# mmziyad/flink-ms

Hardware: AMD Instinct MI355X
Metric: ALS training throughput (ratings/sec per iteration) (higher is better)
Workload: dtype bf16+fp8-factors; 1 GPU; model=ALS-ml25m-shape, rank=64, ratings_per_gpu=25000095, users_per_gpu=162541, num_items=59047, global_batch=25000095, factor_exchange=fp8-e4m3, solve_dtype=fp32, parallelism=dp1+factor-allgather

## Files before the change

flink_ms_amd/ops/csrc/als_kernels.hip:

```cpp

#include "common.hip.h"

#include "als_kernels_device.inc"
#include "fma_api.h"


template <int KT, bool FP8, bool WT = false>
__launch_bounds__(256)
__attribute__((amdgpu_waves_per_eu(3)))
__global__ void k_als_solve_fused(
    const long long* __restrict__ indptr, const int* __restrict__ indices,
    const float* __restrict__ values,
    const typename GatherT<FP8>::elem* __restrict__ factors,
    float* __restrict__ out_f32,
    typename GatherT<FP8>::elem* __restrict__ out_lowp,
    const int* __restrict__ row_order, long long nrows, float reg,
    const float* __restrict__ scale, const float* __restrict__ G0) {
    constexpr int K = Geo<KT>::K;
    __shared__ __align__(16) char
        smem[FP8 ? Geo<KT>::SMEM8_TRI : Geo<KT>::SMEM_TRI];
    long long row = blockIdx.x;
    if (row >= nrows) return;
    if (row_order) row = row_order[row];

// ... 792 lines not shown
            const int row = I * 16 + g4 * 4 + r, col = J * 16 + li;
            if constexpr (I == J)
                T[t][r] = G0[max(row, col) * K + min(row, col)];
            else
                T[t][r] = G0[row * K + col];
        }
        wavefused_load_base<KT, t + 1>(T, G0, g4, li);
    }
}

template <int KT, bool FP8, int BC, bool WT = false>
__launch_bounds__(256)
__attribute__((amdgpu_waves_per_eu(5)))
__global__ void k_als_solve_wavefused(const long long* __restrict__ indptr,
                                      const int* __restrict__ indices,
                                      const float* __restrict__ values,
                                      const void* __restrict__ factors,
                                      float* __restrict__ out_f32,
                                      unsigned short* __restrict__ out_bf16,
                                      unsigned char* __restrict__ out_fp8,
                                      const int* __restrict__ row_order,
                                      long long nrows, float reg,
                                      const float* __restrict__ scale,
                                      const float* __restrict__ G0) {
    constexpr int K = KT * 16;
    static_assert(K <= 64, "wave-fused path handles k <= 64");
    constexpr int NA = KT * (KT + 1) / 2;
    constexpr int TROW = FP8 ? Geo<KT>::TROW8 : Geo<KT>::TROW;
    constexpr int SB = (K + 16) * TROW;
    constexpr int NT = FP8 ? 8 * (K / 16) : K;
    constexpr int NCHW = (2 * NT <= WAVE && NT >= 8) ? 2 : 1;
    constexpr int SCRF = (K * 17 > 1040) ? K * 17 : 1040;
    constexpr int WB0 = (NCHW * SB > SCRF * 4) ? NCHW * SB : SCRF * 4;
    constexpr int WB = (WB0 + 15) & ~15;
    __shared__ __align__(16) char smem[4 * WB];
    const int w = __builtin_amdgcn_readfirstlane(threadIdx.x >> 6);
    const int lane = threadIdx.x & 63;
    const long long e0 = (long long)blockIdx.x * 4 + w;
    if (e0 >= nrows) return;
    const long long e = row_order ? row_order[e0] : e0;
    char* buf = smem + (long long)w * WB;
    float* scr = (float*)buf;
    const int g4 = lane >> 4, li = lane & 15;
    const long long p0 = indptr[e];
    const int n = (int)(indptr[e + 1] - p0);
    if (n == 0) {
        if (lane < K) {
            out_f32[e * K + lane] = 0.0f;
            if (out_bf16) out_bf16[e * K + lane] = 0;
            if (out_fp8) out_fp8[e * K + lane] = 0;
        }
        return;
    }
    {
        constexpr int SEGS = FP8 ? 8 : 16;
        for (int i = lane; i < NCHW * 14 * SEGS; i += WAVE) {
            const int b = i / (14 * SEGS), r2 = i % (14 * SEGS);
            const int row = K + 2 + r2 / SEGS, seg = r2 % SEGS;
            *(unsigned*)(buf + b * SB + (long long)row * TROW + seg * 4) =
                0u;
        }
    }
    f32x4 T[NA], E[KT];
    if constexpr (WT) {
        wavefused_load_base<KT>(T, G0, g4, li);
    } else {
#pragma unroll
        for (int t = 0; t < NA; ++t) T[t] = f32x4{0, 0, 0, 0};
    }
#pragma unroll
    for (int p = 0; p < KT; ++p) E[p] = f32x4{0, 0, 0, 0};
    const int nchunks = (n + 31) >> 5;
    for (int ch = 0; ch < nchunks; ch += NCHW) {
        if constexpr (NCHW == 2) {
            const int sub = (lane >= NT) ? 1 : 0;
            const int lch = ch + sub;
            if (lch < nchunks && lane < 2 * NT)
                stage_chunk_w<KT, FP8, NT, WT>(buf + sub * SB, indices,
                                               values, factors,
                                               p0 + (long long)lch * 32,
                                               n - lch * 32, lane - sub * NT,
                                               scale);
        } else {
            stage_chunk_w<KT, FP8, WAVE, WT>(buf, indices, values, factors,
                                             p0 + (long long)ch * 32,
                                             n - ch * 32, lane, scale);
        }
        WREG_FENCE();
        {
            typename FragT<FP8>::type frag[KT + 1];
            read_frags<KT, FP8>(buf, lane, frag);
            mfma_lower_tiles<KT, FP8>(frag, T);
            mfma_ext_tiles<KT, FP8>(frag, E);
        }
        if constexpr (NCHW == 2) {
            if (ch + 1 < nchunks) {
                typename FragT<FP8>::type frag[KT + 1];
                read_frags<KT, FP8>(buf + SB, lane, frag);
                mfma_lower_tiles<KT, FP8>(frag, T);
                mfma_ext_tiles<KT, FP8>(frag, E);
            }
        }
        WREG_FENCE();
    }
    wavefused_dump_b<KT>(E, scr, g4, li);
    WREG_FENCE();
    float x0 = (lane < K) ? scr[lane] + scr[64 + lane] : 0.0f;
    WREG_FENCE();
    wavefused_diag<KT, BC>(T, reg, (float)n, g4, li);
    float d0 = 1.0f;
    wreg_panels<KT, 0, BC>(T, scr, lane, g4, li, d0);
    const float id0 = wreg_id0<BC>(d0);
    wreg_forward<KT, 0, BC>(T, scr, x0, id0, lane, g4, li);
    x0 *= id0;
    wreg_backward<KT, KT - 1, BC>(T, scr, x0, id0, lane, g4, li);
    x0 = wreg_canon_nan(x0);
    if (lane < K) {
        out_f32[e * K + lane] = x0;
        if (out_bf16) out_bf16[e * K + lane] = f2bf(x0);
        if (out_fp8) out_fp8[e * K + lane] = f2fp8(x0);
    }
}

template <int KT, int t = 0>
DEV_INLINE void factor_gram_store(const f32x4* T, float* dst, int g4, int li) {
    if constexpr (t < KT * (KT + 1) / 2) {
        constexpr int K = KT * 16;
        constexpr int I = lo_tile_i(t);
        constexpr int J = t - (I * (I + 1)) / 2;
#pragma unroll
        for (int r = 0; r < 4; ++r)
            dst[(I * 16 + g4 * 4 + r) * K + J * 16 + li] = T[t][r];
        factor_gram_store<KT, t + 1>(T, dst, g4, li);
    }
}
// ... 427 lines not shown
```

flink_ms_amd/ops/csrc/als_kernels_device.inc:

```
#pragma once

#include <type_traits>


template <int KT> struct Geo {
    static constexpr int K = 16 * KT;
    static constexpr int NA = KT * (KT + 1) / 2;
    static constexpr int TILES = NA + KT;
    static constexpr int SLOTS = (TILES + 3) / 4;
    static constexpr int TROW = 96;
    static constexpr int STAGE_BYTES = (K + 16) * TROW;
    static constexpr int TROW8 = 40;
    static constexpr int STAGE8_BYTES = (K + 16) * TROW8;
    static constexpr int NCH_BF16 = 2;
    static constexpr int NCH_FP8 = 4;
    static constexpr int STAGE_TOTAL = NCH_BF16 * STAGE_BYTES;
    static constexpr int STAGE8_TOTAL = NCH_FP8 * STAGE8_BYTES;
    static constexpr int A_BYTES = K * (K + 1) * 4;
    static constexpr int CHOL_BYTES = A_BYTES + 8 * K + 16 * 16 * 4;
    static constexpr int SMEM = (NCH_BF16 * STAGE_BYTES > CHOL_BYTES)
                                    ? NCH_BF16 * STAGE_BYTES : CHOL_BYTES;
    static constexpr int SMEM8 = (NCH_FP8 * STAGE8_BYTES > CHOL_BYTES)
                                     ? NCH_FP8 * STAGE8_BYTES : CHOL_BYTES;
    static constexpr int LDT = 17;
// ... 25 lines not shown

typedef float stage_f32x2 __attribute__((ext_vector_type(2)));
typedef __bf16 stage_bf16x2 __attribute__((ext_vector_type(2)));

DEV_INLINE float stage_fp8_sat(float x) {
    const unsigned u = __builtin_bit_cast(unsigned, x);
    return (u & 0x7f800000u) != 0x7f800000u
               ? __builtin_amdgcn_fmed3f(x, 448.0f, -448.0f) : x;
}

DEV_INLINE unsigned stage_rescale_fp8x4(unsigned w, float s) {
    const stage_f32x2 s2 = {s, s};
    stage_f32x2 lo = __builtin_amdgcn_cvt_pk_f32_fp8((int)w, false) * s2;
    stage_f32x2 hi = __builtin_amdgcn_cvt_pk_f32_fp8((int)w, true) * s2;
    int r = __builtin_amdgcn_cvt_pk_fp8_f32(stage_fp8_sat(lo.x),
                                            stage_fp8_sat(lo.y), 0, false);
    r = __builtin_amdgcn_cvt_pk_fp8_f32(stage_fp8_sat(hi.x),
                                        stage_fp8_sat(hi.y), r, true);
    return (unsigned)r;
}

DEV_INLINE unsigned stage_rescale_bf16x2(unsigned d, float s) {
    const stage_f32x2 v = {__builtin_bit_cast(float, d << 16),
                           __builtin_bit_cast(float, d & 0xffff0000u)};
    const stage_f32x2 s2 = {s, s};
    return __builtin_bit_cast(
        unsigned, __builtin_convertvector(v * s2, stage_bf16x2));
}

DEV_INLINE uint4 stage_widen_fp8x8(uint2 raw) {
    unsigned out[4];
#pragma unroll
    for (int h = 0; h < 4; ++h) {
        const unsigned w = (h < 2 ? raw.x : raw.y) >> (16 * (h & 1));
        out[h] = (unsigned)f2bf(fp82f((unsigned char)(w & 0xffu)))
                 | ((unsigned)f2bf(fp82f((unsigned char)((w >> 8) & 0xffu)))
                    << 16);
    }
    return uint4{out[0], out[1], out[2], out[3]};
}

template <bool FP8>
DEV_INLINE uint4 stage_rescale_piece(uint4 x, float s) {
    if constexpr (FP8)
        return uint4{stage_rescale_fp8x4(x.x, s), stage_rescale_fp8x4(x.y, s),
                     stage_rescale_fp8x4(x.z, s), stage_rescale_fp8x4(x.w, s)};
    else
        return uint4{stage_rescale_bf16x2(x.x, s),
                     stage_rescale_bf16x2(x.y, s),
                     stage_rescale_bf16x2(x.z, s),
                     stage_rescale_bf16x2(x.w, s)};
}

template <int KT, bool FP8, int NLANES = WAVE, bool WT = false,
          bool IDENT = false, bool WIDEN = false>
DEV_INLINE void stage_chunk_w(char* buf,
                              const int* __restrict__ indices,
                              const float* __restrict__ values,
                              const void* __restrict__ factors_v,
                              long long base, int nrem, int lane,
                              const float* __restrict__ scale = nullptr) {
    constexpr int K = Geo<KT>::K;
    constexpr int TROW = FP8 ? Geo<KT>::TROW8 : Geo<KT>::TROW;
    if constexpr (FP8) {
        const unsigned char* factors = (const unsigned char*)factors_v;
        constexpr int NT = 8 * (K / 16);
        for (int t = lane; t < NT; t += NLANES) {
            const int q = t & 7, c16 = t >> 3;
            uint4 v[4];
            [[maybe_unused]] float sc[4] = {0.0f, 0.0f, 0.0f, 0.0f};
#pragma unroll
            for (int m = 0; m < 4; ++m) {
                uint4 x = {0, 0, 0, 0};
                const int row = 4 * q + m;
                if (row < nrem) {
                    long long col;
                    if constexpr (IDENT) col = base + row;
                    else col = indices[base + row];
                    x = *(const uint4*)(factors + col * (long long)K
                                        + c16 * 16);
                    if constexpr (WT) sc[m] = scale[base + row];
                }
                v[m] = x;
            }
            if constexpr (WT) {
#pragma unroll
                for (int m = 0; m < 4; ++m)
                    v[m] = stage_rescale_piece<FP8>(v[m], sc[m]);
            }
            char* rb = buf + (long long)(16 * c16) * TROW + q * 4;
#pragma unroll
            for (int cc = 0; cc < 16; ++cc) {
                unsigned wd = 0;
#pragma unroll
                for (int m = 0; m < 4; ++m)
                    wd |= (((&v[m].x)[cc >> 2] >> (8 * (cc & 3))) & 0xffu)
                          << (8 * m);
                *(unsigned*)(rb + (long long)cc * TROW) = wd;
            }
        }
    } else {
        const unsigned short* factors = (const unsigned short*)factors_v;
        constexpr int NT = 8 * (K / 8);
        for (int t = lane; t < NT; t += NLANES) {
            const int q = t & 7, c8 = t >> 3;
            uint4 v[4];
            [[maybe_unused]] float sc[4] = {0.0f, 0.0f, 0.0f, 0.0f};
#pragma unroll
            for (int m = 0; m < 4; ++m) {
                uint4 x = {0, 0, 0, 0};
                const int row = 4 * q + m;
                if (row < nrem) {
                    long long col;
                    if constexpr (IDENT) col = base + row;
                    else col = indices[base + row];
                    if constexpr (WIDEN)
                        x = stage_widen_fp8x8(*(const uint2*)(
                            (const unsigned char*)factors_v
                            + col * (long long)K + c8 * 8));
                    else
                        x = *(const uint4*)(factors + col * (long long)K
                                            + c8 * 8);
                    if constexpr (WT) sc[m] = scale[base + row];
                }
                v[m] = x;
            }
            if constexpr (WT) {
#pragma unroll
                for (int m = 0; m < 4; ++m)
                    v[m] = stage_rescale_piece<FP8>(v[m], sc[m]);
            }
            char* rb = buf + (long long)(8 * c8) * TROW + q * 8;
#pragma unroll
            for (int cc = 0; cc < 8; ++cc) {
                const unsigned d0 = (&v[0].x)[cc >> 1], d1 = (&v[1].x)[cc >> 1];
                const unsigned d2 = (&v[2].x)[cc >> 1], d3 = (&v[3].x)[cc >> 1];
                unsigned lo, hi;
                if (cc & 1) {
                    lo = (d0 >> 16) | (d1 & 0xffff0000u);
                    hi = (d2 >> 16) | (d3 & 0xffff0000u);
                } else {
                    lo = (d0 & 0xffffu) | (d1 << 16);
                    hi = (d2 & 0xffffu) | (d3 << 16);
                }
                *(uint2*)(rb + (long long)cc * TROW) = uint2{lo, hi};
            }
        }
    }
    if constexpr (IDENT) return;
    if (lane < 8) {
        if constexpr (FP8) {
            unsigned h = 0, l = 0;
#pragma unroll
            for (int m = 0; m < 4; ++m) {
                const int row = 4 * lane + m;
                const float r = (row < nrem) ? values[base + row] : 0.0f;
                const unsigned char hb = f2fp8(r);
                const unsigned char lb = f2fp8(r - fp82f(hb));
                h |= ((unsigned)hb) << (8 * m);
                l |= ((unsigned)lb) << (8 * m);
            }
            *(unsigned*)(buf + (long long)K * TROW + lane * 4) = h;
            *(unsigned*)(buf + (long long)(K + 1) * TROW + lane * 4) = l;
        } else {
            unsigned h2[2] = {0, 0}, l2[2] = {0, 0};
#pragma unroll
            for (int m = 0; m < 4; ++m) {
                const int row = 4 * lane + m;
                const float r = (row < nrem) ? values[base + row] : 0.0f;
                const unsigned short h = f2bf(r);
                const unsigned short l = f2bf(r - bf2f(h));
                h2[m >> 1] |= ((unsigned)h) << (16 * (m & 1));
                l2[m >> 1] |= ((unsigned)l) << (16 * (m & 1));
            }
            *(uint2*)(buf + (long long)K * TROW + lane * 8) =
                uint2{h2[0], h2[1]};
            *(uint2*)(buf + (long long)(K + 1) * TROW + lane * 8) =
                uint2{l2[0], l2[1]};
        }
    }
}

template <int KT, bool FP8, int NCH>
DEV_INLINE void stage_zero_pad_all(char* smem) {
    constexpr int K = Geo<KT>::K;
    constexpr int TROW = FP8 ? Geo<KT>::TROW8 : Geo<KT>::TROW;
    constexpr int SB = (K + 16) * TROW;
    constexpr int SEGS = FP8 ? 8 : 16;
    for (int i = threadIdx.x; i < NCH * 14 * SEGS; i += 256) {
        const int b = i / (14 * SEGS), rem = i % (14 * SEGS);
        const int row = K + 2 + rem / SEGS, seg = rem % SEGS;
        *(unsigned*)(smem + (long long)b * SB + (long long)row * TROW
                     + seg * 4) = 0u;
    }
}

template <int KT, bool FP8>
DEV_INLINE void read_frags(const char* buf, int lane,
                           typename FragT<FP8>::type* frag) {
    constexpr int TROW = FP8 ? Geo<KT>::TROW8 : Geo<KT>::TROW;
    constexpr int FB = FP8 ? 8 : 16;
    const int g = lane >> 4, li = lane & 15;
#pragma unroll
    for (int t = 0; t <= KT; ++t)
        frag[t] = *(const typename FragT<FP8>::type*)(
            buf + (long long)(t * 16 + li) * TROW + g * FB);
}


template <int KT, int W, bool FP8, int S = 0>
DEV_INLINE void mfma_tiles(const typename FragT<FP8>::type* frag, f32x4* acc) {
    if constexpr (S < Geo<KT>::SLOTS) {
        constexpr int t = W + 4 * S;
        if constexpr (t < Geo<KT>::TILES) {
            constexpr int NA = Geo<KT>::NA;
            constexpr int p = (t < NA) ? up_tile_p(t, KT) : (t - NA);
            constexpr int q = (t < NA) ? up_tile_q((t < NA) ? t : 0, KT) : KT;
            if constexpr (FP8) {
                acc[S] = __builtin_amdgcn_mfma_f32_16x16x32_fp8_fp8(
                    frag[p], frag[q], acc[S], 0, 0, 0);
            } else {
                acc[S] = __builtin_amdgcn_mfma_f32_16x16x32_bf16(
                    frag[p], frag[q], acc[S], 0, 0, 0);
            }
        }
        mfma_tiles<KT, W, FP8, S + 1>(frag, acc);
    }
}

template <int KT, int W, int S = 0>
DEV_INLINE void write_acc(const f32x4* acc, float* A, float* bhi, float* blo,
                          int lane) {
    if constexpr (S < Geo<KT>::SLOTS) {
        constexpr int t = W + 4 * S;
        if constexpr (t < Geo<KT>::TILES) {
            constexpr int K = Geo<KT>::K;
            constexpr int NA = Geo<KT>::NA;
            constexpr int p = (t < NA) ? up_tile_p(t, KT) : (t - NA);
            constexpr int q = (t < NA) ? up_tile_q((t < NA) ? t : 0, KT) : KT;
            const int g = lane >> 4, li = lane & 15;
#pragma unroll
            for (int r = 0; r < 4; ++r) {
                const int row = p * 16 + g * 4 + r;
                if constexpr (q == KT) {
                    if (li == 0) bhi[row] = acc[S][r];
                    else if (li == 1) blo[row] = acc[S][r];
                } else {
// ... 201 lines not shown
        }
        __syncthreads();
        if (own && tid < B0) {
            const float* Tbr = A + tri_off(bi, Ir) * TSZ + lr;
            float s = 0.0f;
#pragma unroll
            for (int cc = 0; cc < 16; ++cc)
                s += Tbr[cc * LDT] * xbuf[B0 + cc];
            acc -= s * invd;
        } else if (own && tid >= B0 && tid < B0 + 16) {
            acc = xbuf[tid];
        }
        __syncthreads();
    }
    if (own) {
        x_row[tid] = acc;
        if (xb_row) xb_row[tid] = f2bf(acc);
        if (x8_row) x8_row[tid] = f2fp8(acc);
    }
}

template <int KT, bool COMBINE = true, bool TRI = false, bool FP8 = false,
          bool WT = false>
DEV_INLINE int gramian_to_lds(char* smem,
                              const long long* __restrict__ indptr,
                              const int* __restrict__ indices,
                              const float* __restrict__ values,
                              const void* __restrict__ factors,
                              long long row, float reg,
                              const float* __restrict__ scale = nullptr,
                              const float* __restrict__ G0 = nullptr) {
    constexpr int K = Geo<KT>::K;
    constexpr int NCH = FP8 ? Geo<KT>::NCH_FP8 : Geo<KT>::NCH_BF16;
    constexpr int SB = (K + 16) * (FP8 ? Geo<KT>::TROW8 : Geo<KT>::TROW);
    const int tid = threadIdx.x, lane = tid & 63;
    const int w = __builtin_amdgcn_readfirstlane(threadIdx.x >> 6);
    const long long p0 = indptr[row];
    const int n = (int)(indptr[row + 1] - p0);
    if (n == 0) return 0;

    f32x4 acc[Geo<KT>::SLOTS];
#pragma unroll
    for (int s = 0; s < Geo<KT>::SLOTS; ++s) acc[s] = f32x4{0, 0, 0, 0};

    constexpr int NT = FP8 ? 8 * (K / 16) : K;
    constexpr int TW = (NT > WAVE) ? 2 : 1;
    constexpr int NCHU = (NCH < 4 / TW) ? NCH : 4 / TW;
    stage_zero_pad_all<KT, FP8, NCHU>(smem);
    const int team = w / TW;
    const int tlane = (w % TW) * WAVE + lane;
    const int nchunks = (n + 31) >> 5;
    for (int r0 = 0; r0 < nchunks; r0 += NCHU) {
        if (team < NCHU && r0 + team < nchunks)
            stage_chunk_w<KT, FP8, TW * WAVE, WT>(
                smem + team * SB, indices, values, factors,
                p0 + (long long)(r0 + team) * 32, n - (r0 + team) * 32,
                tlane, scale);
        __syncthreads();
        const int ns = min(NCHU, nchunks - r0);
        for (int sc = 0; sc < ns; ++sc) {
            typename FragT<FP8>::type frag[KT + 1];
            read_frags<KT, FP8>(smem + sc * SB, lane, frag);
            switch (w) {
                case 0: mfma_tiles<KT, 0, FP8>(frag, acc); break;
                case 1: mfma_tiles<KT, 1, FP8>(frag, acc); break;
                case 2: mfma_tiles<KT, 2, FP8>(frag, acc); break;
                default: mfma_tiles<KT, 3, FP8>(frag, acc); break;
            }
        }
        __syncthreads();
    }

    float* A = (float*)smem;
    float* bhi = A + (TRI ? Geo<KT>::A_TRI_FLOATS : K * (K + 1));
    float* blo = bhi + K;
    if constexpr (TRI) {
        switch (w) {
            case 0: write_acc_tri<KT, 0>(acc, A, bhi, blo, lane); break;
            case 1: write_acc_tri<KT, 1>(acc, A, bhi, blo, lane); break;
            case 2: write_acc_tri<KT, 2>(acc, A, bhi, blo, lane); break;
            default: write_acc_tri<KT, 3>(acc, A, bhi, blo, lane); break;
        }
    } else {
        switch (w) {
            case 0: write_acc<KT, 0>(acc, A, bhi, blo, lane); break;
            case 1: write_acc<KT, 1>(acc, A, bhi, blo, lane); break;
            case 2: write_acc<KT, 2>(acc, A, bhi, blo, lane); break;
            default: write_acc<KT, 3>(acc, A, bhi, blo, lane); break;
        }
    }
    __syncthreads();
    if constexpr (WT && COMBINE) {
        if constexpr (TRI) {
            const int lr = tid >> 4, lc = tid & 15;
            int I = 0, J = 0;
            for (int t = 0; t < Geo<KT>::NA; ++t) {
                const int r = I * 16 + lr, c = J * 16 + lc;
                A[t * Geo<KT>::TSZ + lr * Geo<KT>::LDT + lc] +=
                    G0[max(r, c) * K + min(r, c)];
                if (++J > I) { ++I; J = 0; }
            }
        } else {
            for (int i = tid; i < K * K; i += 256) {
                const int r = i / K, c = i % K;
                A[r * (K + 1) + c] += G0[max(r, c) * K + min(r, c)];
            }
        }
// ... 33 lines not shown
```

flink_ms_amd/ops/csrc/bindings.cpp:

```cpp

#include <torch/extension.h>

#include <charconv>
#include <cstdint>
#include <cstdlib>
#include <thread>
#include <vector>

#include "fma_api.h"

namespace {

py::tuple parse_als_block(py::object text_o, int64_t k) {
    Py_buffer view;
    if (PyObject_GetBuffer(text_o.ptr(), &view, PyBUF_SIMPLE) != 0)
        throw py::error_already_set();
    char* base = (char*)view.buf;
    Py_ssize_t total = view.len;
    std::vector<std::pair<int64_t, int64_t>> lines;
    int64_t start = 0;
    for (int64_t i = 0; i < total; ++i) {
        if (base[i] == '\n') {
            if (i > start) lines.emplace_back(start, i);
            start = i + 1;
// ... 694 lines not shown
              a.name());
    return py::make_tuple(greater, equal, score);
}

int64_t rank_chunk_items(int64_t np, int64_t nc) {
    return (int64_t)fma_rank_chunk_items(np, nc);
}


void mfma_probe_f32(torch::Tensor A, torch::Tensor B, torch::Tensor D,
                    int64_t stream) {
    Args a("mfma_probe_f32");
    a.flat(A, kF32, "A", 16 * 4, true);
    a.flat(B, kF32, "B", 4 * 16, true);
    a.flat(D, kF32, "D", 16 * 16, true);
    check_hip(fma_mfma_probe_f32(f32(A), f32(B), f32(D), a.stream(stream)),
              a.name());
}

void mfma_probe_bf16(torch::Tensor Xt, torch::Tensor Yt, torch::Tensor C,
                     int64_t stream) {
    Args a("mfma_probe_bf16");
    a.flat(Xt, kBF16, "Xt", 32 * 16, true);
    a.flat(Yt, kBF16, "Yt", 32 * 16, true);
    a.flat(C, kF32, "C", 16 * 16, true);
    check_hip(fma_mfma_probe_bf16(bf16(Xt), bf16(Yt), f32(C),
                                  a.stream(stream)),
              a.name());
}

void mfma_probe_fp8(torch::Tensor Xt, torch::Tensor Yt, torch::Tensor C,
                    int64_t stream) {
    Args a("mfma_probe_fp8");
    a.flat(Xt, kU8, "Xt", 32 * 16, true);
    a.flat(Yt, kU8, "Yt", 32 * 16, true);
    a.flat(C, kF32, "C", 16 * 16, true);
    check_hip(fma_mfma_probe_fp8(u8(Xt), u8(Yt), f32(C), a.stream(stream)),
              a.name());
}

void dbg_stage_dump(torch::Tensor indptr, torch::Tensor indices,
                    torch::Tensor values, torch::Tensor factors,
                    torch::Tensor out, int64_t stream) {
    Args a("dbg_stage_dump");
    TORCH_CHECK(a.csr(indptr, indices, values) >= 1, a.name(),
                ": indptr must hold at least one entity");
    const int k = a.factors(factors, false, "factors");
    a.flat(out, kBF16, "out", (int64_t)(k + 16) * 32, false);
    check_hip(fma_dbg_stage_dump(k, i64(indptr), i32(indices), f32(values),
                                 bf16(factors), bf16(out), a.stream(stream)),
              a.name());
}

void dbg_frag_dump(torch::Tensor indptr, torch::Tensor indices,
                   torch::Tensor values, torch::Tensor factors,
                   torch::Tensor out, int64_t stream) {
    Args a("dbg_frag_dump");
    TORCH_CHECK(a.csr(indptr, indices, values) >= 1, a.name(),
                ": indptr must hold at least one entity");
    const int k = a.factors(factors, false, "factors");
    a.flat(out, kBF16, "out", (int64_t)4 * (k / 16 + 1) * 64 * 8,
           false);
    check_hip(fma_dbg_frag_dump(k, i64(indptr), i32(indices), f32(values),
                                bf16(factors), bf16(out), a.stream(stream)),
              a.name());
}

void dbg_gramian(torch::Tensor indptr, torch::Tensor indices,
                 torch::Tensor values, torch::Tensor factors,
                 torch::Tensor A_out, torch::Tensor bhi, torch::Tensor blo,
                 double reg, int64_t stream) {
    Args a("dbg_gramian");
    const int64_t nrows = a.csr(indptr, indices, values);
    const int k = a.factors(factors, false, "factors");
    a.square_rows(A_out, "A_out", nrows, k);
    a.rows(bhi, kF32, "bhi", nrows, k);
    a.rows(blo, kF32, "blo", nrows, k);
    check_hip(fma_dbg_gramian(k, i64(indptr), i32(indices), f32(values),
                              bf16(factors), f32(A_out), f32(bhi), f32(blo),
                              nrows, (float)reg, a.stream(stream)),
              a.name());
}

}

void register_kvserver(pybind11::module_& m);

PYBIND11_MODULE(TORCH_EXTENSION_NAME, m) {
    m.doc() = "flink_ms_amd MI355X (gfx950) HIP kernels";
    register_kvserver(m);
    m.def("als_solve_fused", &als_solve_fused);
    m.def("gramian", &gramian);
    m.attr("BROADCAST_SHFL") = kBroadcastShfl;
    m.attr("BROADCAST_DEFAULT") = kBroadcastDefault;
    m.def("als_solve_wavefused", &als_solve_wavefused, py::arg("indptr"),
          py::arg("indices"), py::arg("values"), py::arg("factors"),
          py::arg("out_f32"), py::arg("out_bf16"), py::arg("out_fp8"),
          py::arg("row_order"), py::arg("reg"), py::arg("stream"),
          py::arg("variant") = kBroadcastDefault);
    m.def("als_solve_wavefused_db", &als_solve_wavefused_db,
          py::arg("indptr"), py::arg("indices"), py::arg("values"),
          py::arg("factors"), py::arg("out_f32"), py::arg("out_bf16"),
          py::arg("out_fp8"), py::arg("row_order"), py::arg("reg"),
          py::arg("stream"), py::arg("variant") = kBroadcastDefault);
    m.def("gramian_w", &gramian_w);
    m.def("als_solve_fused_w", &als_solve_fused_w);
    m.def("als_solve_wavefused_w", &als_solve_wavefused_w);
    m.def("factor_gram", &factor_gram, py::arg("factors"),
          py::arg("rows_per_part"), py::arg("stream"));
    m.def("factor_gram_rows_per_part", &factor_gram_rows_per_part);
    m.def("cholesky_solve", &cholesky_solve);
    m.def("cholesky_solve_ph", &cholesky_solve_ph);
    m.def("ldl_solve_wave", &ldl_solve_wave);
    m.def("ldl_solve_wave_reg", &ldl_solve_wave_reg, py::arg("A"),
          py::arg("b"), py::arg("x"), py::arg("x_bf16"), py::arg("x_fp8"),
          py::arg("stream"), py::arg("variant") = kBroadcastDefault);
    m.def("sdca_pass", &sdca_pass);
    m.def("sdca_num_waves", &sdca_num_waves);
    m.def("svm_margins", &svm_margins);
    m.def("predict_dot", &predict_dot);
    m.def("sgd_update", &sgd_update);
    m.def("topk_scores", &topk_scores, py::arg("Q"), py::arg("V"),
          py::arg("cand"), py::arg("excl_ptr"), py::arg("excl_rows"),
          py::arg("topk"), py::arg("chunk_items"), py::arg("stream"));
    m.def("topk_chunk_items", &topk_chunk_items);
    m.def("rank_counts", &rank_counts, py::arg("Q"), py::arg("V"),
          py::arg("T"), py::arg("q_idx"), py::arg("skip"), py::arg("cand"),
          py::arg("excl_ptr"), py::arg("excl_rows"), py::arg("chunk_items"),
          py::arg("stream"));
    m.def("rank_chunk_items", &rank_chunk_items);
    m.def("dbg_stage_dump", &dbg_stage_dump);
    m.def("dbg_frag_dump", &dbg_frag_dump);
    m.def("dbg_gramian", &dbg_gramian);
    m.def("mfma_probe_f32", &mfma_probe_f32);
    m.def("mfma_probe_bf16", &mfma_probe_bf16);
    m.def("mfma_probe_fp8", &mfma_probe_fp8);
    m.def("parse_als_block", &parse_als_block);
}
```

flink_ms_amd/ops/csrc/debug_kernels.hip:

```cpp

#include "common.hip.h"

#include "als_kernels_device.inc"
#include "fma_api.h"

template <int KT>
__launch_bounds__(256)
__global__ void k_stage_dump(const long long* __restrict__ indptr,
                             const int* __restrict__ indices,
                             const float* __restrict__ values,
                             const unsigned short* __restrict__ factors,
                             unsigned short* __restrict__ out) {
    constexpr int K = Geo<KT>::K;
    constexpr int TROW = Geo<KT>::TROW;
    __shared__ __align__(16) char smem[Geo<KT>::SMEM];
    const long long p0 = indptr[0];
    const int n = (int)(indptr[1] - p0);
    stage_zero_pad_all<KT, false, 1>(smem);
    if (threadIdx.x < 64)
        stage_chunk_w<KT, false>(smem, indices, values, factors, p0, n,
                                 threadIdx.x);
    __syncthreads();
    for (int i = threadIdx.x; i < (K + 16) * 32; i += 256) {
        const int row = i / 32, col = i % 32;
        out[i] = *(const unsigned short*)(smem + (long long)row * TROW
                                          + col * 2);
    }
}

template <int KT>
__launch_bounds__(256)
__global__ void k_frag_dump(const long long* __restrict__ indptr,
                            const int* __restrict__ indices,
                            const float* __restrict__ values,
                            const unsigned short* __restrict__ factors,
                            unsigned short* __restrict__ out) {
    __shared__ __align__(16) char smem[Geo<KT>::SMEM];
    const long long p0 = indptr[0];
    const int n = (int)(indptr[1] - p0);
    stage_zero_pad_all<KT, false, 1>(smem);
    if (threadIdx.x < 64)
        stage_chunk_w<KT, false>(smem, indices, values, factors, p0, n,
                                 threadIdx.x);
    __syncthreads();
    const int lane = threadIdx.x & 63, w = threadIdx.x >> 6;
    bf16x8 frag[KT + 1];
    read_frags<KT, false>(smem, lane, frag);
    for (int t = 0; t <= KT; ++t)
        for (int j = 0; j < 8; ++j)
            out[((w * (KT + 1) + t) * 64 + lane) * 8 + j] =
                (unsigned short)frag[t][j];
}

template <int KT>
__launch_bounds__(256)
__global__ void k_gramian_dbg(const long long* __restrict__ indptr,
                              const int* __restrict__ indices,
                              const float* __restrict__ values,
                              const unsigned short* __restrict__ factors,
                              float* __restrict__ A_out,
                              float* __restrict__ bhi_out,
                              float* __restrict__ blo_out,
                              long long nrows, float reg) {
    constexpr int K = Geo<KT>::K;
    __shared__ __align__(16) char smem[Geo<KT>::SMEM];
    const long long row = blockIdx.x;
    if (row >= nrows) return;
    const int tid = threadIdx.x;
    const int n = gramian_to_lds<KT, false>(
        smem, indptr, indices, values, factors, row, reg);
    float* A = (float*)smem;
    float* bhi = A + K * (K + 1);
    float* blo = bhi + K;
    if (n == 0) return;
    for (int i = tid; i < K * K; i += 256)
        A_out[row * K * K + i] = A[(i / K) * (K + 1) + (i % K)];
    for (int c = tid; c < K; c += 256) {
        bhi_out[row * K + c] = bhi[c];
        blo_out[row * K + c] = blo[c];
    }
}


extern "C" int fma_dbg_stage_dump(
    int k, const long long* indptr, const int* indices, const float* values,
    const unsigned short* factors, unsigned short* out, void* stream) {
    if (k % 16) return hipErrorInvalidValue;
    return dispatch_ic<1, 2, 3, 4, 5, 6, 7, 8>(k / 16, [&](auto kt) {
        k_stage_dump<decltype(kt)::value>
            <<<dim3(1), dim3(256), 0, (hipStream_t)stream>>>(
                indptr, indices, values, factors, out);
        return hipGetLastError();
    });
}

extern "C" int fma_dbg_frag_dump(
    int k, const long long* indptr, const int* indices, const float* values,
    const unsigned short* factors, unsigned short* out, void* stream) {
    if (k % 16) return hipErrorInvalidValue;
    return dispatch_ic<1, 2, 3, 4, 5, 6, 7, 8>(k / 16, [&](auto kt) {
        k_frag_dump<decltype(kt)::value>
            <<<dim3(1), dim3(256), 0, (hipStream_t)stream>>>(
                indptr, indices, values, factors, out);
        return hipGetLastError();
    });
}

extern "C" int fma_dbg_gramian(
    int k, const long long* indptr, const int* indices, const float* values,
    const unsigned short* factors, float* A_out, float* bhi_out,
    float* blo_out, long long nrows, float reg, void* stream) {
    if (k % 16 || nrows <= 0) return hipErrorInvalidValue;
    return dispatch_ic<1, 2, 3, 4, 5, 6, 7, 8>(k / 16, [&](auto kt) {
        k_gramian_dbg<decltype(kt)::value>
            <<<dim3((unsigned)nrows), dim3(256), 0, (hipStream_t)stream>>>(
                indptr, indices, values, factors, A_out, bhi_out, blo_out,
                nrows, reg);
        return hipGetLastError();
    });
}
```

flink_ms_amd/ops/csrc/fma_api.h:

```cpp
#pragma once

#ifdef __cplusplus
extern "C" {
#endif

const char* fma_err_str(int err);

int fma_als_solve_fused(int k, int fp8, const long long* indptr,
                        const int* indices, const float* values,
                        const void* factors, float* out_f32,
                        unsigned short* out_bf16, unsigned char* out_fp8,
                        const int* row_order, long long nrows, float reg,
                        void* stream);
int fma_gramian(int k, int fp8, const long long* indptr, const int* indices,
                const float* values, const void* factors, float* A_out,
                float* b_out, const int* row_order, long long nrows,
                float reg, void* stream);
int fma_cholesky_solve_ph(int k, const float* A_in, const float* b_in,
                          float* x_out, long long nrows, int phases,
                          void* stream);
int fma_cholesky_solve(int k, const float* A_in, const float* b_in,
                       float* x_out, long long nrows, void* stream);

int fma_ldl_solve_wave(int k, const float* A_in, const float* b_in,
// ... 6 lines not shown
int fma_als_solve_wavefused(int k, int fp8, const long long* indptr,
                            const int* indices, const float* values,
                            const void* factors, float* out_f32,
                            unsigned short* out_bf16, unsigned char* out_fp8,
                            const int* row_order, long long nrows, float reg,
                            int variant, void* stream);
int fma_als_solve_wavefused_db(int k, const long long* indptr,
                               const int* indices, const float* values,
                               const void* factors, float* out_f32,
                               unsigned short* out_bf16,
                               unsigned char* out_fp8, const int* row_order,
                               long long nrows, float reg, int variant,
                               void* stream);

int fma_gramian_w(int k, int fp8, const long long* indptr, const int* indices,
                  const float* scale, const float* ext, const float* base,
                  const void* factors, float* A_out, float* b_out,
                  const int* row_order, long long nrows, float reg,
                  void* stream);
int fma_als_solve_fused_w(int k, int fp8, const long long* indptr,
                          const int* indices, const float* scale,
                          const float* ext, const float* base,
                          const void* factors, float* out_f32,
                          unsigned short* out_bf16, unsigned char* out_fp8,
                          const int* row_order, long long nrows, float reg,
                          void* stream);
int fma_als_solve_wavefused_w(int k, int fp8, const long long* indptr,
                              const int* indices, const float* scale,
                              const float* ext, const float* base,
                              const void* factors, float* out_f32,
                              unsigned short* out_bf16,
                              unsigned char* out_fp8, const int* row_order,
                              long long nrows, float reg, void* stream);

int fma_factor_gram(int k, int fp8, const void* factors, long long n,
                    long long rows_per_part, float* G, void* workspace,
                    long long workspace_bytes, void* stream);
long long fma_factor_gram_workspace_bytes(long long n, int k,
                                          long long rows_per_part);
long long fma_factor_gram_rows_per_part(long long n, int k);

int fma_mfma_probe_f32(const float* A , const float* B ,
                       float* D , void* stream);
int fma_mfma_probe_bf16(const unsigned short* Xt ,
                        const unsigned short* Yt ,
                        float* C , void* stream);
int fma_mfma_probe_fp8(const unsigned char* Xt ,
                       const unsigned char* Yt ,
                       float* C , void* stream);

int fma_dbg_stage_dump(int k, const long long* indptr, const int* indices,
                       const float* values, const unsigned short* factors,
                       unsigned short* out , void* stream);
int fma_dbg_frag_dump(int k, const long long* indptr, const int* indices,
                      const float* values, const unsigned short* factors,
                      unsigned short* out ,
                      void* stream);
int fma_dbg_gramian(int k, const long long* indptr, const int* indices,
                    const float* values, const unsigned short* factors,
                    float* A_out, float* bhi_out, float* blo_out,
                    long long nrows, float reg, void* stream);

int fma_sdca_pass(const long long* indptr, const int* indices,
                  const float* values, const float* y, const float* norms_sq,
                  const int* perm, float* alpha, float* v, long long nrows,
                  float scale, void* stream);
long long fma_sdca_num_waves(long long nrows);
int fma_svm_margins(const long long* indptr, const int* indices,
                    const float* values, const float* w, float* out,
                    long long nrows, void* stream);

int fma_predict_dot(const unsigned short* U, const unsigned short* V,
                    const long long* u_idx, const long long* i_idx,
                    float* out, long long nq, int k, void* stream);
int fma_sgd_update(unsigned short* U, unsigned short* V,
                   const long long* u_idx, const long long* i_idx,
                   const float* r, float* err_out, long long nq, int k,
                   float lr, float user_reg, float item_reg, void* stream);

int fma_topk_scores(const unsigned short* Q, const unsigned short* V,
                    const long long* cand, const long long* excl_ptr,
                    const long long* excl_rows, float* out_scores,
                    long long* out_rows, void* workspace,
                    long long workspace_bytes, long long nq, long long nv,
                    long long nc, int k, int topk, long long chunk_items,
                    void* stream);
long long fma_topk_workspace_bytes(long long nq, long long nc, int topk,
                                   long long chunk_items);
long long fma_topk_chunk_items(long long nq, long long nc, int topk);

int fma_rank_counts(const unsigned short* Q, const unsigned short* V,
                    const unsigned short* T, const long long* q_idx,
                    const long long* skip, const long long* cand,
                    const long long* excl_ptr, const long long* excl_rows,
                    long long* greater, long long* equal, float* score,
                    void* workspace, long long workspace_bytes, long long np,
                    long long nq, long long nv, long long nc, int k,
                    long long chunk_items, void* stream);
long long fma_rank_workspace_bytes(long long np, long long nc,
                                   long long chunk_items);
long long fma_rank_chunk_items(long long np, long long nc);

#ifdef __cplusplus
}
#endif
```

Before: 16.54 billion ratings/s.

## Restructure ALS chunk staging with fast-path gathers and per-lane rating encode

Splits chunk staging into a gather part and a ratings part. When a chunk is full, indices are read with one 16-byte vector load and the factor rows are gathered without per-row bounds checks. Each lane now loads one rating early and encodes it after the gather, so the latency of the values load overlaps the factor loads. The fp8 byte transpose now uses permute instructions, pad zeroing uses 16-byte stores, and an fp8 stage-dump debug entry point is added. Register pressure may rise, and the separate code paths add complexity.

```diff
diff --git a/flink_ms_amd/ops/csrc/als_kernels.hip b/flink_ms_amd/ops/csrc/als_kernels.hip
--- a/flink_ms_amd/ops/csrc/als_kernels.hip
+++ b/flink_ms_amd/ops/csrc/als_kernels.hip
@@ -868,15 +868,9 @@
         }
         return;
     }
-    {
-        constexpr int SEGS = FP8 ? 8 : 16;
-        for (int i = lane; i < NCHW * 14 * SEGS; i += WAVE) {
-            const int b = i / (14 * SEGS), r2 = i % (14 * SEGS);
-            const int row = K + 2 + r2 / SEGS, seg = r2 % SEGS;
-            *(unsigned*)(buf + b * SB + (long long)row * TROW + seg * 4) =
-                0u;
-        }
-    }
+#pragma unroll
+    for (int b = 0; b < NCHW; ++b)
+        stage_zero_pad<KT, FP8>(buf + b * SB, lane, WAVE);
     f32x4 T[NA], E[KT];
     if constexpr (WT) {
         wavefused_load_base<KT>(T, G0, g4, li);
@@ -889,14 +883,17 @@
     const int nchunks = (n + 31) >> 5;
     for (int ch = 0; ch < nchunks; ch += NCHW) {
         if constexpr (NCHW == 2) {
+            const int rem = n - ch * 32;
+            const bool full = rem >= 64;
+            const long long cb = p0 + (long long)ch * 32;
+            const float xr = stage_ext_load(values, cb, rem, lane, full);
             const int sub = (lane >= NT) ? 1 : 0;
-            const int lch = ch + sub;
-            if (lch < nchunks && lane < 2 * NT)
-                stage_chunk_w<KT, FP8, NT, WT>(buf + sub * SB, indices,
-                                               values, factors,
-                                               p0 + (long long)lch * 32,
-                                               n - lch * 32, lane - sub * NT,
-                                               scale);
+            if (2 * NT == WAVE || lane < 2 * NT)
+                stage_gather_w<KT, FP8, NT, WT>(buf + sub * SB, indices,
+                                                factors, cb, rem,
+                                                lane - sub * NT, 32 * sub,
+                                                full, scale);
+            stage_ext_commit<KT, FP8>(buf + (lane >> 5) * SB, lane & 31, xr);
         } else {
             stage_chunk_w<KT, FP8, WAVE, WT>(buf, indices, values, factors,
                                              p0 + (long long)ch * 32,
diff --git a/flink_ms_amd/ops/csrc/als_kernels_device.inc b/flink_ms_amd/ops/csrc/als_kernels_device.inc
--- a/flink_ms_amd/ops/csrc/als_kernels_device.inc
+++ b/flink_ms_amd/ops/csrc/als_kernels_device.inc
@@ -101,37 +101,80 @@
                      stage_rescale_bf16x2(x.w, s)};
 }
 
+#define STAGE_NO_SINK() asm volatile("")
+
+template <int ROWB, bool WT, bool IDENT, bool WIDEN>
+DEV_INLINE void stage_gather4(uint4 (&v)[4], float (&sc)[4],
+                              const int* __restrict__ indices,
+                              const char* __restrict__ factors,
+                              const float* __restrict__ scale,
+                              long long base, int nrem, int row0, int coff,
+                              bool full) {
+    if constexpr (!IDENT && !WIDEN) {
+        if (full) {
+            int idx[4];
+            __builtin_memcpy(idx, indices + base + (unsigned)row0, 16);
+            if constexpr (WT)
+                __builtin_memcpy(sc, scale + base + (unsigned)row0, 16);
+#pragma unroll
+            for (int m = 0; m < 4; ++m)
+                v[m] = *(const uint4*)(factors + (long long)idx[m] * ROWB
+                                       + coff);
+            STAGE_NO_SINK();
+            return;
+        }
+    }
+#pragma unroll
+    for (int m = 0; m < 4; ++m) {
+        uint4 x = {0, 0, 0, 0};
+        const int row = row0 + m;
+        if (row < nrem) {
+            long long col;
+            if constexpr (IDENT) col = base + row;
+            else col = indices[base + (unsigned)row];
+            if constexpr (WIDEN)
+                x = stage_widen_fp8x8(
+                    *(const uint2*)(factors + col * (long long)ROWB + coff));
+            else
+                x = *(const uint4*)(factors + col * (long long)ROWB + coff);
+            if constexpr (WT) sc[m] = scale[base + (unsigned)row];
+        }
+        v[m] = x;
+    }
+}
+
+DEV_INLINE void stage_transpose4x4_b8(unsigned a0, unsigned a1, unsigned a2,
+                                      unsigned a3, unsigned* out) {
+    const unsigned p01l = __builtin_amdgcn_perm(a1, a0, 0x05010400u);
+    const unsigned p01h = __builtin_amdgcn_perm(a1, a0, 0x07030602u);
+    const unsigned p23l = __builtin_amdgcn_perm(a3, a2, 0x05010400u);
+    const unsigned p23h = __builtin_amdgcn_perm(a3, a2, 0x07030602u);
+    out[0] = __builtin_amdgcn_perm(p23l, p01l, 0x05040100u);
+    out[1] = __builtin_amdgcn_perm(p23l, p01l, 0x07060302u);
+    out[2] = __builtin_amdgcn_perm(p23h, p01h, 0x05040100u);
+    out[3] = __builtin_amdgcn_perm(p23h, p01h, 0x07060302u);
+}
+
 template <int KT, bool FP8, int NLANES = WAVE, bool WT = false,
           bool IDENT = false, bool WIDEN = false>
-DEV_INLINE void stage_chunk_w(char* buf,
-                              const int* __restrict__ indices,
-                              const float* __restrict__ values,
-                              const void* __restrict__ factors_v,
-                              long long base, int nrem, int lane,
-                              const float* __restrict__ scale = nullptr) {
+DEV_INLINE void stage_gather_w(char* buf,
+                               const int* __restrict__ indices,
+                               const void* __restrict__ factors_v,
+                               long long base, int nrem, int lane, int crow0,
+                               bool full,
+                               const float* __restrict__ scale = nullptr) {
     constexpr int K = Geo<KT>::K;
     constexpr int TROW = FP8 ? Geo<KT>::TROW8 : Geo<KT>::TROW;
+    const char* factors = (const char*)factors_v;
     if constexpr (FP8) {
-        const unsigned char* factors = (const unsigned char*)factors_v;
         constexpr int NT = 8 * (K / 16);
         for (int t = lane; t < NT; t += NLANES) {
             const int q = t & 7, c16 = t >> 3;
             uint4 v[4];
             [[maybe_unused]] float sc[4] = {0.0f, 0.0f, 0.0f, 0.0f};
-#pragma unroll
-            for (int m = 0; m < 4; ++m) {
-                uint4 x = {0, 0, 0, 0};
-                const int row = 4 * q + m;
-                if (row < nrem) {
-                    long long col;
-                    if constexpr (IDENT) col = base + row;
-                    else col = indices[base + row];
-                    x = *(const uint4*)(factors + col * (long long)K
-                                        + c16 * 16);
-                    if constexpr (WT) sc[m] = scale[base + row];
-                }
-                v[m] = x;
-            }
+            stage_gather4<K, WT, IDENT, false>(v, sc, indices, factors, scale,
+                                               base, nrem, crow0 + 4 * q,
+                                               c16 * 16, full);
             if constexpr (WT) {
 #pragma unroll
                 for (int m = 0; m < 4; ++m)
@@ -139,41 +182,24 @@
             }
             char* rb = buf + (long long)(16 * c16) * TROW + q * 4;
 #pragma unroll
-            for (int cc = 0; cc < 16; ++cc) {
-                unsigned wd = 0;
-#pragma unroll
-                for (int m = 0; m < 4; ++m)
-                    wd |= (((&v[m].x)[cc >> 2] >> (8 * (cc & 3))) & 0xffu)
-                          << (8 * m);
-                *(unsigned*)(rb + (long long)cc * TROW) = wd;
+            for (int d = 0; d < 4; ++d) {
+                unsigned wd[4];
+                stage_transpose4x4_b8((&v[0].x)[d], (&v[1].x)[d],
+                                      (&v[2].x)[d], (&v[3].x)[d], wd);
+#pragma unroll
+                for (int c = 0; c < 4; ++c)
+                    *(unsigned*)(rb + (long long)(4 * d + c) * TROW) = wd[c];
             }
         }
     } else {
-        const unsigned short* factors = (const unsigned short*)factors_v;
         constexpr int NT = 8 * (K / 8);
         for (int t = lane; t < NT; t += NLANES) {
             const int q = t & 7, c8 = t >> 3;
             uint4 v[4];
             [[maybe_unused]] float sc[4] = {0.0f, 0.0f, 0.0f, 0.0f};
-#pragma unroll
-            for (int m = 0; m < 4; ++m) {
-                uint4 x = {0, 0, 0, 0};
-                const int row = 4 * q + m;
-                if (row < nrem) {
-                    long long col;
-                    if constexpr (IDENT) col = base + row;
-                    else col = indices[base + row];
-                    if constexpr (WIDEN)
-                        x = stage_widen_fp8x8(*(const uint2*)(
-                            (const unsigned char*)factors_v
-                            + col * (long long)K + c8 * 8));
-                    else
-                        x = *(const uint4*)(factors + col * (long long)K
-                                            + c8 * 8);
-                    if constexpr (WT) sc[m] = scale[base + row];
-                }
-                v[m] = x;
-            }
+            stage_gather4<(WIDEN ? K : 2 * K), WT, IDENT, WIDEN>(
+                v, sc, indices, factors, scale, base, nrem, crow0 + 4 * q,
+                WIDEN ? c8 * 8 : c8 * 16, full);
             if constexpr (WT) {
 #pragma unroll
                 for (int m = 0; m < 4; ++m)
@@ -196,38 +222,111 @@
             }
         }
     }
-    if constexpr (IDENT) return;
-    if (lane < 8) {
-        if constexpr (FP8) {
-            unsigned h = 0, l = 0;
-#pragma unroll
-            for (int m = 0; m < 4; ++m) {
-                const int row = 4 * lane + m;
-                const float r = (row < nrem) ? values[base + row] : 0.0f;
-                const unsigned char hb = f2fp8(r);
-                const unsigned char lb = f2fp8(r - fp82f(hb));
-                h |= ((unsigned)hb) << (8 * m);
-                l |= ((unsigned)lb) << (8 * m);
-            }
-            *(unsigned*)(buf + (long long)K * TROW + lane * 4) = h;
-            *(unsigned*)(buf + (long long)(K + 1) * TROW + lane * 4) = l;
-        } else {
-            unsigned h2[2] = {0, 0}, l2[2] = {0, 0};
-#pragma unroll
-            for (int m = 0; m < 4; ++m) {
-                const int row = 4 * lane + m;
-                const float r = (row < nrem) ? values[base + row] : 0.0f;
-                const unsigned short h = f2bf(r);
-                const unsigned short l = f2bf(r - bf2f(h));
-                h2[m >> 1] |= ((unsigned)h) << (16 * (m & 1));
-                l2[m >> 1] |= ((unsigned)l) << (16 * (m & 1));
-            }
-            *(uint2*)(buf + (long long)K * TROW + lane * 8) =
-                uint2{h2[0], h2[1]};
-            *(uint2*)(buf + (long long)(K + 1) * TROW + lane * 8) =
-                uint2{l2[0], l2[1]};
-        }
-    }
+}
+
+DEV_INLINE float stage_ext_load(const float* __restrict__ values,
+                                long long base, int nrem, int row,
+                                bool full) {
+    float x = 0.0f;
+    if (full) {
+        x = values[base + (unsigned)row];
+        STAGE_NO_SINK();
+    } else if (row < nrem) {
+        x = values[base + (unsigned)row];
+    }
+    return x;
+}
+
+template <int KT, bool FP8>
+DEV_INLINE void stage_ext_commit(char* buf, int r, float x) {
+    constexpr int K = Geo<KT>::K;
+    constexpr int TROW = FP8 ? Geo<KT>::TROW8 : Geo<KT>::TROW;
+    if constexpr (FP8) {
+        const unsigned char hb = f2fp8(x);
+        const unsigned char lb = f2fp8(x - fp82f(hb));
+        *(unsigned char*)(buf + (long long)K * TROW + r) = hb;
+        *(unsigned char*)(buf + (long long)(K + 1) * TROW + r) = lb;
+    } else {
+        const unsigned short h = f2bf(x);
+        const unsigned short l = f2bf(x - bf2f(h));
+        *(unsigned short*)(buf + (long long)K * TROW + r * 2) = h;
+        *(unsigned short*)(buf + (long long)(K + 1) * TROW + r * 2) = l;
+    }
+}
+
+template <int KT, bool FP8>
+DEV_INLINE void stage_ext_quad_w(char* buf, const float* __restrict__ values,
+                                 long long base, int nrem, int lane) {
+    constexpr int K = Geo<KT>::K;
+    constexpr int TROW = FP8 ? Geo<KT>::TROW8 : Geo<KT>::TROW;
+    if constexpr (FP8) {
+        unsigned h = 0, l = 0;
+#pragma unroll
+        for (int m = 0; m < 4; ++m) {
+            const int row = 4 * lane + m;
+            const float r = (row < nrem) ? values[base + row] : 0.0f;
+            const unsigned char hb = f2fp8(r);
+            const unsigned char lb = f2fp8(r - fp82f(hb));
+            h |= ((unsigned)hb) << (8 * m);
+            l |= ((unsigned)lb) << (8 * m);
+        }
+        *(unsigned*)(buf + (long long)K * TROW + lane * 4) = h;
+        *(unsigned*)(buf + (long long)(K + 1) * TROW + lane * 4) = l;
+    } else {
+        unsigned h2[2] = {0, 0}, l2[2] = {0, 0};
+#pragma unroll
+        for (int m = 0; m < 4; ++m) {
+            const int row = 4 * lane + m;
+            const float r = (row < nrem) ? values[base + row] : 0.0f;
+            const unsigned short h = f2bf(r);
+            const unsigned short l = f2bf(r - bf2f(h));
+            h2[m >> 1] |= ((unsigned)h) << (16 * (m & 1));
+            l2[m >> 1] |= ((unsigned)l) << (16 * (m & 1));
+        }
+        *(uint2*)(buf + (long long)K * TROW + lane * 8) = uint2{h2[0], h2[1]};
+        *(uint2*)(buf + (long long)(K + 1) * TROW + lane * 8) =
+            uint2{l2[0], l2[1]};
+    }
+}
+
+template <int KT, bool FP8, int NLANES = WAVE, bool WT = false,
+          bool IDENT = false, bool WIDEN = false, bool WIDE = false,
+          bool EXT8 = false>
+DEV_INLINE void stage_chunk_w(char* buf,
+                              const int* __restrict__ indices,
+                              const float* __restrict__ values,
+                              const void* __restrict__ factors_v,
+                              long long base, int nrem, int lane,
+                              const float* __restrict__ scale = nullptr) {
+    static_assert(NLANES >= 32, "the EXT rows take 32 lanes");
+    const bool full = WIDE && !IDENT && nrem >= 32;
+    [[maybe_unused]] float xr = 0.0f;
+    if constexpr (!IDENT && EXT8) {
+        static_assert(!WIDE, "EXT8 goes with the guarded gather");
+        if (lane < 8) stage_ext_quad_w<KT, FP8>(buf, values, base, nrem, lane);
+    } else if constexpr (!IDENT) {
+        if (lane < 32) {
+            xr = stage_ext_load(values, base, nrem, lane, full);
+            if constexpr (!WIDE) stage_ext_commit<KT, FP8>(buf, lane, xr);
+        }
+    }
+    stage_gather_w<KT, FP8, NLANES, WT, IDENT, WIDEN>(
+        buf, indices, factors_v, base, nrem, lane, 0, full, scale);
+    if constexpr (!IDENT && WIDE) {
+        if (lane < 32) stage_ext_commit<KT, FP8>(buf, lane, xr);
+    }
+}
+
+template <int KT, bool FP8>
+DEV_INLINE void stage_zero_pad(char* buf, int i, int stride) {
+    constexpr int K = Geo<KT>::K;
+    constexpr int TROW = FP8 ? Geo<KT>::TROW8 : Geo<KT>::TROW;
+    constexpr int N16 = 14 * TROW / 16;
+    static_assert((14 * TROW) % 16 == 0 && ((K + 2) * TROW) % 16 == 0,
+                  "pad rows must be a 16-byte-aligned range");
+    char* pad = buf + (long long)(K + 2) * TROW;
+    for (; i < N16; i += stride)
+        *(uint4*)(pad + (long long)i * 16) = uint4{0u, 0u, 0u, 0u};
 }
 
 template <int KT, bool FP8, int NCH>
@@ -235,13 +334,9 @@
     constexpr int K = Geo<KT>::K;
     constexpr int TROW = FP8 ? Geo<KT>::TROW8 : Geo<KT>::TROW;
     constexpr int SB = (K + 16) * TROW;
-    constexpr int SEGS = FP8 ? 8 : 16;
-    for (int i = threadIdx.x; i < NCH * 14 * SEGS; i += 256) {
-        const int b = i / (14 * SEGS), rem = i % (14 * SEGS);
-        const int row = K + 2 + rem / SEGS, seg = rem % SEGS;
-        *(unsigned*)(smem + (long long)b * SB + (long long)row * TROW
-                     + seg * 4) = 0u;
-    }
+#pragma unroll
+    for (int b = 0; b < NCH; ++b)
+        stage_zero_pad<KT, FP8>(smem + (long long)b * SB, threadIdx.x, 256);
 }
 
 template <int KT, bool FP8>
@@ -549,7 +644,8 @@
     const int nchunks = (n + 31) >> 5;
     for (int r0 = 0; r0 < nchunks; r0 += NCHU) {
         if (team < NCHU && r0 + team < nchunks)
-            stage_chunk_w<KT, FP8, TW * WAVE, WT>(
+            stage_chunk_w<KT, FP8, TW * WAVE, WT, false, false, false,
+                          (!FP8 && KT == 7)>(
                 smem + team * SB, indices, values, factors,
                 p0 + (long long)(r0 + team) * 32, n - (r0 + team) * 32,
                 tlane, scale);
diff --git a/flink_ms_amd/ops/csrc/bindings.cpp b/flink_ms_amd/ops/csrc/bindings.cpp
--- a/flink_ms_amd/ops/csrc/bindings.cpp
+++ b/flink_ms_amd/ops/csrc/bindings.cpp
@@ -770,6 +770,20 @@
               a.name());
 }
 
+void dbg_stage_dump_fp8(torch::Tensor indptr, torch::Tensor indices,
+                        torch::Tensor values, torch::Tensor factors,
+                        torch::Tensor out, int64_t stream) {
+    Args a("dbg_stage_dump_fp8");
+    TORCH_CHECK(a.csr(indptr, indices, values) >= 1, a.name(),
+                ": indptr must hold at least one entity");
+    const int k = a.factors(factors, true, "factors");
+    a.flat(out, kU8, "out", (int64_t)(k + 16) * 32, false);
+    check_hip(fma_dbg_stage_dump_fp8(k, i64(indptr), i32(indices),
+                                     f32(values), u8(factors), u8(out),
+                                     a.stream(stream)),
+              a.name());
+}
+
 void dbg_frag_dump(torch::Tensor indptr, torch::Tensor indices,
                    torch::Tensor values, torch::Tensor factors,
                    torch::Tensor out, int64_t stream) {
@@ -848,6 +862,7 @@
           py::arg("stream"));
     m.def("rank_chunk_items", &rank_chunk_items);
     m.def("dbg_stage_dump", &dbg_stage_dump);
+    m.def("dbg_stage_dump_fp8", &dbg_stage_dump_fp8);
     m.def("dbg_frag_dump", &dbg_frag_dump);
     m.def("dbg_gramian", &dbg_gramian);
     m.def("mfma_probe_f32", &mfma_probe_f32);
diff --git a/flink_ms_amd/ops/csrc/debug_kernels.hip b/flink_ms_amd/ops/csrc/debug_kernels.hip
--- a/flink_ms_amd/ops/csrc/debug_kernels.hip
+++ b/flink_ms_amd/ops/csrc/debug_kernels.hip
@@ -4,27 +4,33 @@
 #include "als_kernels_device.inc"
 #include "fma_api.h"
 
-template <int KT>
+template <int KT, bool FP8>
 __launch_bounds__(256)
 __global__ void k_stage_dump(const long long* __restrict__ indptr,
                              const int* __restrict__ indices,
                              const float* __restrict__ values,
-                             const unsigned short* __restrict__ factors,
-                             unsigned short* __restrict__ out) {
+                             const typename GatherT<FP8>::elem* __restrict__
+                                 factors,
+                             typename GatherT<FP8>::elem* __restrict__ out) {
+    using elem = typename GatherT<FP8>::elem;
     constexpr int K = Geo<KT>::K;
-    constexpr int TROW = Geo<KT>::TROW;
-    __shared__ __align__(16) char smem[Geo<KT>::SMEM];
+    constexpr int TROW = FP8 ? Geo<KT>::TROW8 : Geo<KT>::TROW;
+    constexpr int SB = (K + 16) * TROW;
+    __shared__ __align__(16) char smem[SB];
     const long long p0 = indptr[0];
     const int n = (int)(indptr[1] - p0);
-    stage_zero_pad_all<KT, false, 1>(smem);
+    for (int i = threadIdx.x; i < SB / 4; i += 256)
+        ((unsigned*)smem)[i] = 0xA5A5A5A5u;
+    __syncthreads();
+    stage_zero_pad_all<KT, FP8, 1>(smem);
     if (threadIdx.x < 64)
-        stage_chunk_w<KT, false>(smem, indices, values, factors, p0, n,
-                                 threadIdx.x);
+        stage_chunk_w<KT, FP8, WAVE, false, false, false, true>(
+            smem, indices, values, factors, p0, n, threadIdx.x);
     __syncthreads();
     for (int i = threadIdx.x; i < (K + 16) * 32; i += 256) {
         const int row = i / 32, col = i % 32;
-        out[i] = *(const unsigned short*)(smem + (long long)row * TROW
-                                          + col * 2);
+        out[i] = *(const elem*)(smem + (long long)row * TROW
+                                + col * sizeof(elem));
     }
 }
 
@@ -87,7 +93,19 @@
     const unsigned short* factors, unsigned short* out, void* stream) {
     if (k % 16) return hipErrorInvalidValue;
     return dispatch_ic<1, 2, 3, 4, 5, 6, 7, 8>(k / 16, [&](auto kt) {
-        k_stage_dump<decltype(kt)::value>
+        k_stage_dump<decltype(kt)::value, false>
+            <<<dim3(1), dim3(256), 0, (hipStream_t)stream>>>(
+                indptr, indices, values, factors, out);
+        return hipGetLastError();
+    });
+}
+
+extern "C" int fma_dbg_stage_dump_fp8(
+    int k, const long long* indptr, const int* indices, const float* values,
+    const unsigned char* factors, unsigned char* out, void* stream) {
+    if (k % 16) return hipErrorInvalidValue;
+    return dispatch_ic<1, 2, 3, 4, 5, 6, 7, 8>(k / 16, [&](auto kt) {
+        k_stage_dump<decltype(kt)::value, true>
             <<<dim3(1), dim3(256), 0, (hipStream_t)stream>>>(
                 indptr, indices, values, factors, out);
         return hipGetLastError();
diff --git a/flink_ms_amd/ops/csrc/fma_api.h b/flink_ms_amd/ops/csrc/fma_api.h
--- a/flink_ms_amd/ops/csrc/fma_api.h
+++ b/flink_ms_amd/ops/csrc/fma_api.h
@@ -82,6 +82,9 @@
 int fma_dbg_stage_dump(int k, const long long* indptr, const int* indices,
                        const float* values, const unsigned short* factors,
                        unsigned short* out , void* stream);
+int fma_dbg_stage_dump_fp8(int k, const long long* indptr, const int* indices,
+                           const float* values, const unsigned char* factors,
+                           unsigned char* out , void* stream);
 int fma_dbg_frag_dump(int k, const long long* indptr, const int* indices,
                       const float* values, const unsigned short* factors,
                       unsigned short* out ,
```

Result: faster. 18.81 billion ratings/s, median of 6 (+13.7%).
